# blindopen/TSM-Det-Pointcloud-

Measured on AMD Instinct MI355X. Metric: point-cloud frames/sec (fwd+bwd), higher is better.
Workload: dtype f32; 1 GPU; BASELINE configs[1]: KITTI-shaped synthetic, 20000 pts / 16000 active voxels per frame, full SECOND detector (VoxelBackBone8x) fwd+bwd+AdamW step; batch_per_gpu=4, global_batch=4, parallelism=dp1, voxelize_on_gpu=True

## Files before the change

include/spx.h:

```cpp
#ifndef SPX_H_
#define SPX_H_

#include <stddef.h>
#include <stdint.h>

#ifdef __cplusplus
extern "C" {
#endif

#define SPX_ABI_VERSION 3

#define SPX_OK 0
#define SPX_ERR_INVALID_ARG (-1)
#define SPX_ERR_WORKSPACE (-2)
#define SPX_ERR_UNSUPPORTED (-3)
#define SPX_ERR_LAUNCH (-4)
#define SPX_ERR_TOO_LARGE (-5)
#define SPX_ERR_CAPACITY (-7)
#define SPX_ERR_TABLE_FULL (-6)
#define SPX_ERR_RING_STALL (-8)
#define SPX_ERR_BATCH_STATS (-10)
#define SPX_ERR_OUT_OF_GRID (-9)

#define SPX_WS_PRECLEARED 1
// ... 83 lines not shown
int spx_densify_bwd(const float *ddense, const int32_t *idx, int64_t n, const int64_t *d_n, int c, int batch,
                    const int32_t *shape, int layout, float *dfeat, spx_stream_t stream);

int spx_boxes_iou_bev(const float *boxes_a, int64_t n, const float *boxes_b, int64_t m, int overlap_only, float *out,
                      spx_stream_t stream);
size_t spx_nms_ws_bytes(int64_t n);
int spx_nms_bev(const float *boxes, int64_t n, float thresh, int axis_aligned, int64_t *keep, int64_t *d_num_keep,
                void *ws, size_t ws_bytes, spx_stream_t stream);

size_t spx_assign_targets_ws_bytes(int batch, int n_sets, int max_gt);
int spx_assign_targets(const float *anchors, int n_sets, int64_t anchors_per_set, int per_location,
                       const float *gt_boxes, int batch, int max_gt, const int32_t *d_set_class, int n_classes,
                       const float *d_matched, const float *d_unmatched, int32_t *labels, float *targets,
                       float *weights, void *ws, size_t ws_bytes, spx_stream_t stream);

size_t spx_anchor_loss_ws_bytes(int batch, int64_t n_anchors);
int spx_anchor_loss(const float *cls_preds, const float *box_preds, const float *dir_preds, const int32_t *labels,
                    const float *reg_targets, const float *anchors, int batch, int64_t n_anchors, int num_class,
                    int num_dir_bins, float dir_offset, float cls_weight, float loc_weight, float dir_weight,
                    float beta, float alpha, float *losses, float *dcls, float *dbox, float *ddir, void *ws,
                    size_t ws_bytes, spx_stream_t stream);

size_t spx_bn_relu_ws_bytes(int c);
int spx_bn_relu_fwd(const float *x, int64_t n, const int64_t *d_n, int c, const float *gamma, const float *beta,
                    float *running_mean, float *running_var, float momentum, float eps, int relu, float *y,
                    float *save_mean, float *save_invstd, void *ws, size_t ws_bytes, spx_stream_t stream);
int spx_bn_relu_bwd(const float *x, const float *dy, int64_t n, const int64_t *d_n, int c, const float *gamma, const float *beta,
                    const float *save_mean, const float *save_invstd, int relu, float *dx, float *dgamma, float *dbeta,
                    void *ws, size_t ws_bytes, spx_stream_t stream);

int spx_bn_add_relu_fwd(const float *x, const float *res, int64_t n, const int64_t *d_n, int c, const float *gamma,
                        const float *beta, float *running_mean, float *running_var, int64_t *num_batches_tracked,
                        float momentum, float eps, int relu, float *y, int64_t y_ld, float *save_mean, float *save_invstd,
                        void *ws, size_t ws_bytes, spx_stream_t stream);
int spx_bn_add_relu_bwd(const float *x, const float *res, const float *dy, int64_t dy_ld, int64_t n, const int64_t *d_n,
                        int c, const float *gamma, const float *beta, const float *save_mean, const float *save_invstd, int relu,
                        float *dx, float *dres, float *dgamma, float *dbeta, void *ws, size_t ws_bytes,
                        spx_stream_t stream);

int spx_bn_apply(const float *x, const float *res, int64_t n, const int64_t *d_n, int c, const float *mean,
                 const float *invstd, const float *gamma, const float *beta, int relu, float *y, int64_t y_ld,
                 spx_stream_t stream);

int spx_bn_relu_fwd_from_sums(const float *x, int64_t n, const int64_t *d_n, int c, const float *partial, int64_t nblk,
                              const float *gamma,
                              const float *beta, float *running_mean, float *running_var, int64_t *num_batches_tracked,
                              float momentum, float eps, int relu, float *y, int64_t y_ld, float *save_mean,
                              float *save_invstd, spx_stream_t stream);

int64_t spx_wino_stat_rows(int32_t n, int32_t h, int32_t w);
int64_t spx_wino_weight_floats(int32_t cin, int32_t cout);
int spx_wino_weight(const float *w, int64_t s_o, int64_t s_i, int64_t s_a, int64_t s_b, int32_t cin, int32_t cout, int flip,
                    float *u, spx_stream_t stream);
int spx_conv2d_wino(const float *x, int64_t x_ld, const float *u, int32_t n, int32_t h, int32_t w, int32_t cin, int32_t cout,
                    const float *scale, const float *shift, int relu, float *y, int64_t y_ld, float *stat_partials,
                    spx_stream_t stream);

size_t spx_wino_wgrad_ws_bytes(int32_t cin, int32_t cout);
int spx_conv2d_wino_wgrad(const float *x, int64_t x_ld, const float *dy, int64_t dy_ld, int32_t n, int32_t h, int32_t w,
                          int32_t cin, int32_t cout, float *dw, int64_t s_o, int64_t s_i, int64_t s_a, int64_t s_b, void *ws,
                          size_t ws_bytes, spx_stream_t stream);

int spx_voxel_query(const float *new_xyz, const float *xyz, const int32_t *new_coords, const int32_t *point_indices,
                    int64_t m, int batch, const int32_t *shape3, int nsample, float radius, const int32_t *range3,
                    int32_t *idx, int32_t *cnt_unique, spx_stream_t stream);

int spx_voxel_query_dilated(const float *new_xyz, const float *xyz, const int32_t *new_coords,
                            const int32_t *point_indices, int64_t m, int batch, const int32_t *shape3, int nsample,
                            float former_radius, float radius, const int32_t *range3, const int32_t *stride3,
                            int32_t *idx, int32_t *cnt_unique, int32_t *idx_cnt, spx_stream_t stream);


size_t spx_furthest_point_sample_ws_bytes(int32_t b, int64_t n);
int spx_furthest_point_sample(const float *xyz, const float *weights, int32_t b, int64_t n, int32_t npoint, int32_t *idx,
                              void *ws, size_t ws_bytes, spx_stream_t stream);

size_t spx_furthest_point_sample_matrix_ws_bytes(int32_t b, int64_t n);
int spx_furthest_point_sample_matrix(const float *matrix, const float *weights, int32_t b, int64_t n, int32_t npoint,
                                     int32_t *idx, void *ws, size_t ws_bytes, spx_stream_t stream);

int spx_ball_query(const float *xyz, const float *new_xyz, int32_t b, int64_t n, int64_t m, float r_in, float r_out,
                   int32_t nsample, int32_t *idx_cnt, int32_t *idx, spx_stream_t stream);

int spx_group_points(const float *features, const int32_t *idx, int32_t b, int32_t c, int64_t n, int64_t m,
                     int32_t nsample, float *out, spx_stream_t stream);

size_t spx_group_points_bwd_ws_bytes(int32_t b, int64_t n, int64_t m, int32_t nsample);
int spx_group_points_bwd(const float *grad_out, const int32_t *idx, int32_t b, int32_t c, int64_t n, int64_t m,
                         int32_t nsample, float *grad_features, void *ws, size_t ws_bytes, spx_stream_t stream);

int spx_three_nn(const float *unknown, const float *known, int32_t b, int64_t n, int64_t m, float *dist2, int32_t *idx,
                 spx_stream_t stream);

int spx_three_interpolate(const float *features, const int32_t *idx, const float *weight, int32_t b, int32_t c, int64_t m,
                          int64_t n, float *out, spx_stream_t stream);
size_t spx_three_interpolate_bwd_ws_bytes(int32_t b, int64_t m, int64_t n);
int spx_three_interpolate_bwd(const float *grad_out, const int32_t *idx, const float *weight, int32_t b, int32_t c,
                              int64_t m, int64_t n, float *grad_features, void *ws, size_t ws_bytes, spx_stream_t stream);


int spx_points_in_boxes(const float *pts, const float *boxes, int32_t b, int64_t m, int64_t t, int32_t *box_idx,
                        spx_stream_t stream);

size_t spx_roiaware_pool3d_ws_bytes(int64_t n, int64_t np, int32_t ox, int32_t oy, int32_t oz);
int spx_roiaware_pool3d_fwd(const float *rois, const float *pts, const float *feats, int64_t n, int64_t np, int32_t c,
                            int32_t ox, int32_t oy, int32_t oz, int32_t max_pts, int32_t mode, float *pooled,
// ... 199 lines not shown
```

tsm-det-pointcloud-_amd/csrc/wino_conv2d.hip:

```cpp
#include "spx_common.h"

namespace {

typedef float f32x16 __attribute__((ext_vector_type(16)));
typedef float f32x4 __attribute__((ext_vector_type(4)));
typedef float f32x2 __attribute__((ext_vector_type(2)));
typedef unsigned int u32x4 __attribute__((ext_vector_type(4)));

constexpr int kTiles = 32;
constexpr int kKc = 8;
constexpr int kSc = 16;
constexpr int kCoWg = 128;
constexpr int kThreads = 512;
constexpr int kPosFloats = kCoWg * kKc;
constexpr int kPlane = kTiles * kKc + 8;

struct WinoArgs {
  const float* x;
  const float* u;
  float* y;
  const float* scale;
  const float* shift;
  float* stats;
  int64_t x_ld, y_ld;
  uint32_t x_bytes, u_bytes;
  int32_t n, h, w, cin, cout;
  int32_t tiles_x, tiles_y;
  int64_t n_tiles;
  int32_t relu;
  int32_t n_blocks;
};

constexpr int qp(int a, int b, int c, int d) { return a | (b << 2) | (c << 4) | (d << 6); }

__device__ __forceinline__ float dpp_p(float v) {
  return __builtin_bit_cast(float, __builtin_amdgcn_mov_dpp(__builtin_bit_cast(int, v), qp(0, 1, 2, 1), 0xF, 0xF, true));
}
__device__ __forceinline__ float dpp_q(float v) {
  return __builtin_bit_cast(float, __builtin_amdgcn_mov_dpp(__builtin_bit_cast(int, v), qp(2, 2, 1, 3), 0xF, 0xF, true));
}

__host__ __device__ constexpr int wino_channel(int chunk, int slot) {
  return (chunk >> 1) * kSc + (slot >> 1) * 4 + (chunk & 1) * 2 + (slot & 1);
}

__global__ void k_wino_weight(const float* __restrict__ w, int64_t s_o, int64_t s_i, int64_t s_a, int64_t s_b, int cin,
                              int cout, int flip, float* __restrict__ u) {
  const int64_t idx = (int64_t)blockIdx.x * blockDim.x + threadIdx.x;
  const int64_t total = (int64_t)cin * cout;
  if (idx >= total) return;
  const int nchunk = cin / kKc;
  const int sidx = (int)(idx & 3);
  const int col = (int)((idx >> 2) & 31);
  const int hh = (int)((idx >> 7) & 1);
  const int nb = (int)((idx >> 8) & 3);
  const int chunk = (int)((idx >> 10) % nchunk);
  const int cb = (int)((idx >> 10) / nchunk);
  const int ci = wino_channel(chunk, 4 * hh + sidx), co = cb * kCoWg + nb * 32 + col;
  float g[3][3];
#pragma unroll
  for (int a = 0; a < 3; ++a)
#pragma unroll
    for (int b = 0; b < 3; ++b)
      g[a][b] = flip ? w[(int64_t)ci * s_o + (int64_t)co * s_i + (2 - a) * s_a + (2 - b) * s_b]
                     : w[(int64_t)co * s_o + (int64_t)ci * s_i + a * s_a + b * s_b];
  float t[4][3];
#pragma unroll
  for (int b = 0; b < 3; ++b) {
    t[0][b] = g[0][b];
    t[1][b] = 0.5f * (g[0][b] + g[1][b] + g[2][b]);
    t[2][b] = 0.5f * (g[0][b] - g[1][b] + g[2][b]);
    t[3][b] = g[2][b];
  }
  float* dst = u + ((int64_t)(cb * nchunk + chunk) * 16) * kPosFloats + (idx & 1023);
#pragma unroll
  for (int i = 0; i < 4; ++i) {
    dst[(int64_t)(i * 4 + 0) * kPosFloats] = t[i][0];
    dst[(int64_t)(i * 4 + 1) * kPosFloats] = 0.5f * (t[i][0] + t[i][1] + t[i][2]);
    dst[(int64_t)(i * 4 + 2) * kPosFloats] = 0.5f * (t[i][0] - t[i][1] + t[i][2]);
    dst[(int64_t)(i * 4 + 3) * kPosFloats] = t[i][2];
  }
}

template <int NB>
__global__ void __launch_bounds__(kThreads) __attribute__((amdgpu_waves_per_eu(NB == 1 ? 4 : 2, NB == 1 ? 4 : 2)))
k_wino_conv(WinoArgs a) {
  constexpr int kCoW = 64 * NB;
  constexpr int kSmemFloats = 4 * kTiles * kCoW > 2 * 16 * kPlane ? 4 * kTiles * kCoW : 2 * 16 * kPlane;
  __shared__ __attribute__((aligned(16))) float smem[kSmemFloats];

  const int tid = threadIdx.x;
  const int lane = tid & 63;
  const int wave = tid >> 6;
  const int wrow = wave & 3;
  const int half = wave >> 2;
  const int l31 = lane & 31, lh = lane >> 5;

  const int ncb = a.cout / kCoW;
  const int xcd = blockIdx.x & 7, rest = blockIdx.x >> 3;
  const int per = (a.n_blocks + 7) >> 3;
  const int cbw = rest % ncb;
  const int bid = xcd * per + rest / ncb;
  if (bid >= a.n_blocks) return;
  const int64_t tile0 = (int64_t)bid * kTiles;
  const int nbg = (cbw * 2 + half) * NB;
  const int nchunk = a.cin / kKc;
  const int nsuper = a.cin / kSc;

  const int ld_col = tid & 3;
  const int ld_g = (tid >> 2) & 3;
  const int ld_tile = tid >> 4;
  const __amdgpu_buffer_rsrc_t rs_x =
      __builtin_amdgcn_make_buffer_rsrc(const_cast<float*>(a.x), 0, (int)a.x_bytes, 0x00020000);
  const __amdgpu_buffer_rsrc_t rs_u =
      __builtin_amdgcn_make_buffer_rsrc(const_cast<float*>(a.u), 0, (int)a.u_bytes, 0x00020000);
  uint32_t xoff[4];
  {
    const int64_t t = tile0 + ld_tile;
    const bool tv = t < a.n_tiles;
    const int64_t tt = tv ? t : 0;
    const int tx = (int)(tt % a.tiles_x);
    const int ty = (int)((tt / a.tiles_x) % a.tiles_y);
    const int nn = (int)(tt / ((int64_t)a.tiles_x * a.tiles_y));
    const int px = 2 * tx - 1 + ld_col;
#pragma unroll
    for (int i = 0; i < 4; ++i) {
      const int py = 2 * ty - 1 + i;
      const bool ok = tv && px >= 0 && px < a.w && py >= 0 && py < a.h;
      const int64_t pix = ((int64_t)nn * a.h + py) * a.w + px;
      xoff[i] = ok ? (uint32_t)((pix * a.x_ld + ld_g * 4) * 4) : 0xFFFFFFF0u;
    }
  }
  const float sgn = (ld_col == 1) ? 1.0f : -1.0f;
  float* const vdst = smem + ld_col * kPlane + ld_tile * kKc + ld_g * 2;
// ... 123 lines not shown
        f32x4 y1 = (r1 - r2 - r3) * sc4 + sh4;
        if (a.stats) {
          const float m0 = (px < a.w) ? 1.f : 0.f, m1 = (px < a.w && 2 * ty + 1 < a.h) ? 1.f : 0.f;
          st_s += y0 * m0 + y1 * m1;
          st_q += y0 * y0 * m0 + y1 * y1 * m1;
        }
        if (a.relu) {
#pragma unroll
          for (int e = 0; e < 4; ++e) {
            y0[e] = fmaxf(y0[e], 0.f);
            y1[e] = fmaxf(y1[e], 0.f);
          }
        }
        if (px < a.w) {
          const int py = 2 * ty;
          float* dst = a.y + (((int64_t)nn * a.h + py) * a.w + px) * a.y_ld + co0;
          *reinterpret_cast<f32x4*>(dst) = y0;
          if (py + 1 < a.h) *reinterpret_cast<f32x4*>(dst + (int64_t)a.w * a.y_ld) = y1;
        }
      }
    }
    if (c2 == 0) __syncthreads();
  }
  if (a.stats) {
    __syncthreads();
    float* red = smem;
    *reinterpret_cast<f32x4*>(red + (o_t * kQuads + o_q) * 8) = st_s;
    *reinterpret_cast<f32x4*>(red + (o_t * kQuads + o_q) * 8 + 4) = st_q;
    __syncthreads();
    if (tid < kCoW) {
      const int q = tid >> 2, e = tid & 3;
      float s1 = 0.f, s2 = 0.f;
      for (int t = 0; t < kTilesPass; ++t) {
        s1 += red[(t * kQuads + q) * 8 + e];
        s2 += red[(t * kQuads + q) * 8 + 4 + e];
      }
      float* dst = a.stats + (int64_t)bid * 2 * a.cout + cbw * kCoW + tid;
      dst[0] = s1;
      dst[a.cout] = s2;
    }
  }
}

}

extern "C" int64_t spx_wino_weight_floats(int32_t cin, int32_t cout) { return (int64_t)16 * cin * cout; }

extern "C" int spx_wino_weight(const float* w, int64_t s_o, int64_t s_i, int64_t s_a, int64_t s_b, int32_t cin, int32_t cout,
                               int flip, float* u, spx_stream_t stream) {
  if (cin <= 0 || cout <= 0 || cin % kSc != 0 || cout % kCoWg != 0) return SPX_ERR_INVALID_ARG;
  const int64_t total = (int64_t)cin * cout;
  hipLaunchKernelGGL(k_wino_weight, dim3((unsigned)((total + 255) / 256)), dim3(256), 0, spx_s(stream), w, s_o, s_i, s_a,
                     s_b, cin, cout, flip, u);
  SPX_CHECK_LAUNCH();
  return SPX_OK;
}

extern "C" int64_t spx_wino_stat_rows(int32_t n, int32_t h, int32_t w) {
  const int64_t tiles = (int64_t)n * ((w + 1) / 2) * ((h + 1) / 2);
  return (tiles + kTiles - 1) / kTiles;
}

extern "C" int spx_conv2d_wino(const float* x, int64_t x_ld, const float* u, int32_t n, int32_t h, int32_t w, int32_t cin,
                               int32_t cout, const float* scale, const float* shift, int relu, float* y, int64_t y_ld,
                               float* stat_partials, spx_stream_t stream) {
  if (n <= 0 || h <= 0 || w <= 0) return SPX_OK;
  if (cin % kSc != 0 || cout % kCoWg != 0 || x_ld < cin || y_ld < cout || (x_ld & 3) || (y_ld & 3)) return SPX_ERR_INVALID_ARG;
  const int64_t x_bytes = ((int64_t)n * h * w - 1) * x_ld * 4 + (int64_t)cin * 4, u_bytes = (int64_t)16 * cin * cout * 4;
  if (x_bytes >= 0xFFFFFFF0ll || u_bytes >= 0x7FFFFFFFll) return SPX_ERR_TOO_LARGE;
  WinoArgs a;
  a.x = x; a.u = u; a.y = y; a.scale = scale; a.shift = shift; a.stats = stat_partials;
  a.x_ld = x_ld; a.y_ld = y_ld;
  a.x_bytes = (uint32_t)x_bytes; a.u_bytes = (uint32_t)u_bytes;
  a.n = n; a.h = h; a.w = w; a.cin = cin; a.cout = cout;
  a.tiles_x = (w + 1) / 2; a.tiles_y = (h + 1) / 2;
  a.n_tiles = (int64_t)n * a.tiles_x * a.tiles_y;
  a.relu = relu;
  const int64_t nb = (a.n_tiles + kTiles - 1) / kTiles;
  if (nb > 0x7fffffff) return SPX_ERR_INVALID_ARG;
  a.n_blocks = (int32_t)nb;
#ifdef WINO_FORCE_NB
  const bool narrow = WINO_FORCE_NB == 1;
#else
  const bool narrow = true;
#endif
  const int64_t nb8 = (nb + 7) / 8 * 8;
  if (narrow)
    hipLaunchKernelGGL(k_wino_conv<1>, dim3((unsigned)(nb8 * (cout / 64))), dim3(kThreads), 0, spx_s(stream), a);
  else
    hipLaunchKernelGGL(k_wino_conv<2>, dim3((unsigned)(nb8 * (cout / 128))), dim3(kThreads), 0, spx_s(stream), a);
  SPX_CHECK_LAUNCH();
  return SPX_OK;
}
```

tsm-det-pointcloud-_amd/pcdet_amd/models/backbones_2d/base_bev_backbone.py:

```python
import os

import numpy as np
import torch
import torch.nn as nn
import torch.nn.functional as F

from spx import ops

from ..model_utils import det_wgrad
from spx.functional import (bn_relu_cat_train, bn_relu_train, dense as densify_rows, folded_bn, sparse_conv, wino_conv2d,
                            wino_conv2d_ok, wino_conv_bn_relu_train)

_FUSED_BN_MIN_ELEMS = int(os.environ.get("SPX_BEV_FUSED_BN_MIN", str(8 * 1000 * 1000)))


def _run_block(seq, x, start=0):
    mods = list(seq)
    i = start
    while i < len(mods):
        m = mods[i]
        nxt = mods[i + 1] if i + 1 < len(mods) else None
        if (isinstance(m, nn.ZeroPad2d) and isinstance(nxt, nn.Conv2d) and tuple(nxt.padding) == (0, 0)
                and nxt.padding_mode == 'zeros' and len(set(m.padding)) == 1 and isinstance(nxt.padding, tuple)):
            p = int(m.padding[0])
            if det_wgrad.usable(x, nxt):
                x = det_wgrad.conv2d(x, nxt, p)
            else:
                x = F.conv2d(x, nxt.weight, nxt.bias, nxt.stride, (p, p), nxt.dilation, nxt.groups)
            i += 2
            continue
        if _WINO and isinstance(m, nn.Conv2d) and wino_conv2d_ok(x, m):
            nn2 = mods[i + 2] if i + 2 < len(mods) else None
            if (_CONV_BN_NODE and isinstance(nxt, nn.BatchNorm2d) and isinstance(nn2, nn.ReLU) and _train_bn_ok(nxt)
                    and torch.is_grad_enabled()
                    and x.shape[0] * x.shape[2] * x.shape[3] * m.out_channels >= _FUSED_BN_MIN_ELEMS
                    and 1024 % m.out_channels == 0):
                x = wino_conv_bn_relu_train(x, m, nxt)
                i += 3
            elif nxt is not None and isinstance(nn2, nn.ReLU) and _eval_bn_ok(nxt, x, check_layout=False):
                scale, shift, _ = folded_bn(nxt)
                x = wino_conv2d(x, m.weight, scale=scale, shift=shift, relu=True)
                i += 3
            else:
                x = wino_conv2d(x, m.weight)
                i += 1
            continue
        if (isinstance(m, nn.BatchNorm2d) and isinstance(nxt, nn.ReLU) and m.training and m.affine
                and m.track_running_stats and m.momentum is not None and x.is_cuda and x.dtype == torch.float32
                and x.numel() >= _FUSED_BN_MIN_ELEMS and 1024 % x.shape[1] == 0 and x.shape[1] % 4 == 0
                and x.is_contiguous(memory_format=torch.channels_last)):
            b, c, h, w = x.shape
            y = bn_relu_train(x.permute(0, 2, 3, 1).reshape(b * h * w, c), m, True)
            x = y.view(b, h, w, c).permute(0, 3, 1, 2)
            i += 2
            continue
        if _eval_bn_ok(m, x) and isinstance(nxt, nn.ReLU):
            b, c, h, w = x.shape
            y = _bn_eval_rows(x.permute(0, 2, 3, 1).reshape(b * h * w, c), m, True)
            x = y.view(b, h, w, c).permute(0, 3, 1, 2)
            i += 2
            continue
        x = _up(m, x) if isinstance(m, nn.ConvTranspose2d) else m(x)
        i += 1
    return x


def _up(m, x):
    return det_wgrad.conv_transpose2d(x, m) if det_wgrad.usable(x, m) else m(x)


_FUSED_EVAL_BN = os.environ.get("SPX_BEV_FUSED_EVAL_BN", "1") != "0"


_WINO = os.environ.get("SPX_BEV_WINOGRAD", "1") != "0"
_CONV_BN_NODE = os.environ.get("SPX_BEV_CONV_BN_NODE", "1") != "0"


def _train_bn_ok(m):
    return m.training and m.affine and m.track_running_stats and m.momentum is not None and m.weight.dtype == torch.float32


def _eval_bn_ok(m, x, check_layout=True):
    return (_FUSED_EVAL_BN and isinstance(m, nn.BatchNorm2d) and not m.training and m.affine and m.running_mean is not None
            and not torch.is_grad_enabled() and x.is_cuda and x.dtype == torch.float32 and x.dim() == 4
            and not torch.is_autocast_enabled()
            and (not check_layout or (1024 % x.shape[1] == 0 and x.shape[1] % 4 == 0
                                      and x.is_contiguous(memory_format=torch.channels_last))))


def _bn_eval_rows(rows, bn, relu, out=None):
    _scale, _shift, invstd = folded_bn(bn)
    return ops.bn_apply(rows, bn.running_mean, invstd, bn.weight, bn.bias, relu, out=out)


_SPARSE_ENTRY = os.environ.get("SPX_BEV_SPARSE_ENTRY", "1") != "0"
_FUSED_CAT = os.environ.get("SPX_BEV_FUSED_CAT", "1") != "0"
_WIDE_BALANCED = os.environ.get("SPX_BEV_WIDE_BALANCED", "1") != "0"
_SPARSE_ENTRY_CHANNELS = (16, 32, 64, 128)


def _sparse_entry(seq, bev):
    tag = getattr(bev, '_spx_source', None)
    mods = list(seq)
    if not _SPARSE_ENTRY or tag is None or tag[1] != bev._version or len(mods) < 2:
        return None
    src = tag[0]
    pad, conv = mods[0], mods[1]
    if not (isinstance(pad, nn.ZeroPad2d) and isinstance(conv, nn.Conv2d) and len(set(pad.padding)) == 1
            and tuple(conv.padding) == (0, 0) and conv.padding_mode == 'zeros' and conv.bias is None and conv.groups == 1
            and tuple(conv.dilation) == (1, 1) and conv.stride[0] == conv.stride[1]):
        return None
    feats = src.features
    c, d = feats.shape[1], int(src.spatial_shape[0])
    kh, kw = conv.kernel_size
    if not (feats.is_cuda and feats.dtype == torch.float32 and bev.dtype == torch.float32
            and not torch.is_autocast_enabled() and conv.in_channels == c * d and d * kh * kw <= 30
            and c in _SPARSE_ENTRY_CHANNELS and conv.out_channels in _SPARSE_ENTRY_CHANNELS and feats.shape[0] > 0):
# ... 36 lines not shown
        self.blocks = nn.ModuleList()
        self.deblocks = nn.ModuleList()
        for idx in range(num_levels):
            c_out = num_filters[idx]
            layers = [nn.ZeroPad2d(1),
                      nn.Conv2d(c_in_list[idx], c_out, kernel_size=3, stride=layer_strides[idx], padding=0, bias=False),
                      bn(c_out), nn.ReLU()]
            for _ in range(layer_nums[idx]):
                layers += [nn.Conv2d(c_out, c_out, kernel_size=3, padding=1, bias=False), bn(c_out), nn.ReLU()]
            self.blocks.append(nn.Sequential(*layers))
            if len(upsample_strides) > 0:
                stride = upsample_strides[idx]
                if stride >= 1:
                    up = nn.ConvTranspose2d(c_out, num_upsample_filters[idx], stride, stride=stride, bias=False)
                else:
                    s = int(np.round(1 / stride))
                    up = nn.Conv2d(c_out, num_upsample_filters[idx], s, stride=s, bias=False)
                self.deblocks.append(nn.Sequential(up, bn(num_upsample_filters[idx]), nn.ReLU()))

        c_in = sum(num_upsample_filters)
        if len(upsample_strides) > num_levels:
            self.deblocks.append(nn.Sequential(
                nn.ConvTranspose2d(c_in, c_in, upsample_strides[-1], stride=upsample_strides[-1], bias=False),
                bn(c_in), nn.ReLU()))
        self.num_bev_features = c_in
        self.num_voxel_neck_features = c_in
        self.num_point_features = kwargs.get('num_point_features', None)

    def _cat_fusable(self):
        if not _FUSED_CAT or len(self.deblocks) != len(self.blocks) or len(self.deblocks) < 2:
            return False
        for d in self.deblocks:
            mods = list(d)
            if not (len(mods) == 3 and isinstance(mods[1], nn.BatchNorm2d) and isinstance(mods[2], nn.ReLU)
                    and mods[1].training and mods[1].affine and mods[1].track_running_stats and mods[1].momentum is not None
                    and 1024 % mods[1].num_features == 0 and mods[1].num_features % 4 == 0):
                return False
        return True

    def _cat_eval_fusable(self, x):
        if not _FUSED_EVAL_BN or len(self.deblocks) != len(self.blocks) or len(self.deblocks) < 2 or torch.is_grad_enabled():
            return False
        return all(len(d) == 3 and isinstance(d[1], nn.BatchNorm2d) and isinstance(d[2], nn.ReLU) and not d[1].training
                   and d[1].affine and d[1].running_mean is not None and 1024 % d[1].num_features == 0
                   and d[1].num_features % 4 == 0 for d in self.deblocks)

    def forward(self, data_dict):
        spatial_features = data_dict['spatial_features']
        ups, pre = [], []
        x = spatial_features
        plain = x.is_cuda and x.dtype == torch.float32 and not torch.is_autocast_enabled()
        fuse_cat = self._cat_fusable() and plain
        fuse_cat_eval = (not fuse_cat) and plain and self._cat_eval_fusable(x)
        for i in range(len(self.blocks)):
            y = _sparse_entry(self.blocks[i], x) if i == 0 else None
            x = _run_block(self.blocks[i], x) if y is None else _run_block(self.blocks[i], y, start=2)
            stride = int(spatial_features.shape[2] / x.shape[2])
            data_dict['spatial_features_%dx' % stride] = x
            if fuse_cat or fuse_cat_eval:
                pre.append(_up(self.deblocks[i][0], x))
            else:
                ups.append(_run_block(self.deblocks[i], x) if len(self.deblocks) > 0 else x)
        if fuse_cat or fuse_cat_eval:
            b, _c, h, w = pre[0].shape
            same = all(t.shape[0] == b and t.shape[2:] == pre[0].shape[2:]
                       and t.is_contiguous(memory_format=torch.channels_last) for t in pre)
            if same and fuse_cat and all(t.numel() >= _FUSED_BN_MIN_ELEMS for t in pre):
                rows = [t.permute(0, 2, 3, 1).reshape(b * h * w, t.shape[1]) for t in pre]
                y = bn_relu_cat_train(rows, [d[1] for d in self.deblocks])
                ups = [y.view(b, h, w, y.shape[1]).permute(0, 3, 1, 2)]
            elif same and fuse_cat_eval:
                widths = [t.shape[1] for t in pre]
                y = torch.empty((b * h * w, sum(widths)), dtype=torch.float32, device=x.device)
                off = 0
                for t, d, wd in zip(pre, self.deblocks, widths):
                    _bn_eval_rows(t.permute(0, 2, 3, 1).reshape(b * h * w, wd), d[1], True, out=y[:, off:off + wd])
                    off += wd
                ups = [y.view(b, h, w, y.shape[1]).permute(0, 3, 1, 2)]
            else:
                ups = [_run_block(d, t, start=1) for d, t in zip(self.deblocks, pre)]
        if len(ups) > 1:
            x = torch.cat(ups, dim=1)
        elif len(ups) == 1:
            x = ups[0]
        if len(self.deblocks) > len(self.blocks):
            x = _run_block(self.deblocks[-1], x)
        data_dict['spatial_features_2d'] = x
        data_dict['encoded_bev_features'] = [x]
        return data_dict
```

tsm-det-pointcloud-_amd/spx/_lib.py:

```python
import ctypes
import os

import torch

_HERE = os.path.dirname(os.path.abspath(__file__))
LIB_PATH = os.environ.get("SPX_LIB_PATH") or os.path.join(os.path.dirname(_HERE), "csrc", "libspx.so")

SPX_ABI_VERSION = 3
SPX_MAX_KVOL = 32

_vp = ctypes.c_void_p
_i64 = ctypes.c_int64
_int = ctypes.c_int
_sz = ctypes.c_size_t
_i32p = ctypes.POINTER(ctypes.c_int32)
_f32p = ctypes.POINTER(ctypes.c_float)
_vpp = ctypes.POINTER(ctypes.c_void_p)

class PointMlp(ctypes.Structure):
    _fields_ = [("w1", _vp), ("bn_mean", _vp), ("bn_var", _vp), ("bn_weight", _vp), ("bn_bias", _vp),
                ("bn_eps", ctypes.c_float), ("w2", _vp), ("b2", _vp)]


_mlpp = ctypes.POINTER(PointMlp)
# ... 5 lines not shown
    "spx_read_status": (_int, [_vp, _vp]),
    "spx_voxelize": (_int, [_vp, _i64, _int, _int, _int, _int, _int, _int, _f32p, _f32p, _i32p, _int, _int, _vp, _vp,
                            _vp, _vp, _vp, _i64, _int, _vp, _vp, _sz, _vp]),
    "spx_dynamic_voxelize_ws_bytes": (_sz, [_i64, _int, _i32p, _i64]),
    "spx_dynamic_voxelize": (_int, [_vp, _i64, _int, _int, _int, _int, _f32p, _f32p, _i32p, _int, _vp, _vp, _vp, _vp, _i64,
                                    _vp, _sz, _vp]),
    "spx_voxel_query": (_int, [_vp, _vp, _vp, _vp, _i64, _int, _i32p, _int, ctypes.c_float, _i32p, _vp, _vp, _vp]),
    "spx_voxel_query_dilated": (_int, [_vp, _vp, _vp, _vp, _i64, _int, _i32p, _int, ctypes.c_float, ctypes.c_float, _i32p,
                                       _i32p, _vp, _vp, _vp, _vp]),
    "spx_mean_vfe": (_int, [_vp, _vp, _i64, _vp, _int, _int, _vp, _vp]),
    "spx_subm_rulebook_ws_bytes": (_sz, [_i64]),
    "spx_subm_rulebook": (_int, [_vp, _i64, _vp, _int, _i32p, _i32p, _i32p, _vp, _i64, _vp, _int, _vp, _vp, _sz, _vp]),
    "spx_conv_out_cap": (_i64, [_i64, _int, _i32p, _i32p, _i32p]),
    "spx_conv_rulebook_ws_bytes": (_sz, [_i64, _int, _i32p]),
    "spx_conv_rulebook": (_int, [_vp, _i64, _vp, _int, _i32p, _i32p, _i32p, _i32p, _i32p, _i32p, _vp, _vp, _vp, _vp,
                                 _vp, _i64, _i32p, _i32p, _vp, _vp, _vp, _vp, _sz, _vp]),
    "spx_pack_weight": (_int, [_vp, _int, _int, _int, _int, _vp, _vp]),
    "spx_pack_weight_batched": (_int, [_vp, _int, _i64, _vp]),
    "spx_conv_gemm": (_int, [_vp, _int, _vp, _int, _int, _int, _vp, _i64, _i64, _vp, _vp, _vp, _int, _vp, _vp]),
    "spx_conv_plan_bytes": (_sz, [_i64]),
    "spx_conv_plan": (_int, [_vp, _i64, _int, _i64, _vp, _vp, _vp]),
    "spx_conv_gemm_balanced_ws_bytes": (_sz, [_int, _i64]),
    "spx_conv_group_ws_bytes": (_sz, [_i64]),
    "spx_conv_group": (_int, [_vp, _i64, _int, _i64, _vp, _vp, _vp, _vp, _sz, _vp]),
    "spx_conv_gemm_balanced": (_int, [_vp, _int, _vp, _int, _int, _int, _vp, _i64, _i64, _vp, _vp, _vp, _int, _vp, _vp, _vp,
                                      _vp, _sz, _vp]),
    "spx_conv_ring_plan_bytes": (_sz, [_i64]),
    "spx_conv_ring_stat_rows": (_int, []),
    "spx_conv_ring_tiles_per_wave": (_int, [_int]),
    "spx_conv_ring_plan": (_int, [_vp, _i64, _int, _i64, _vp, _vp, _vp]),
    "spx_conv_gemm_ring": (_int, [_vp, _i64, _int, _vp, _int, _int, _int, _vp, _i64, _i64, _vp, _vp, _vp, _int, _vp, _vp, _vp,
                                  _vp, _vp, _vp]),
    "spx_conv_wgrad_ws_bytes": (_sz, [_int, _int, _int, _i64]),
    "spx_conv_wgrad_counts_bytes": (_sz, [_int, _i64]),
    "spx_conv_wgrad_counts": (_int, [_vp, _i64, _int, _i64, _vp, _vp, _vp]),
    "spx_conv_wgrad": (_int, [_vp, _int, _vp, _int, _int, _vp, _i64, _i64, _vp, _vp, _vp, _vp, _sz, _vp]),
    "spx_densify": (_int, [_vp, _vp, _i64, _vp, _int, _int, _i32p, _int, _vp, _vp]),
    "spx_densify_bwd": (_int, [_vp, _vp, _i64, _vp, _int, _int, _i32p, _int, _vp, _vp]),
    "spx_boxes_iou_bev": (_int, [_vp, _i64, _vp, _i64, _int, _vp, _vp]),
    "spx_nms_ws_bytes": (_sz, [_i64]),
    "spx_nms_bev": (_int, [_vp, _i64, ctypes.c_float, _int, _vp, _vp, _vp, _sz, _vp]),
    "spx_assign_targets_ws_bytes": (_sz, [_int, _int, _int]),
    "spx_bn_relu_ws_bytes": (_sz, [_int]),
    "spx_bn_relu_fwd": (_int, [_vp, _i64, _vp, _int, _vp, _vp, _vp, _vp, ctypes.c_float, ctypes.c_float, _int, _vp, _vp,
                               _vp, _vp, _sz, _vp]),
    "spx_bn_relu_bwd": (_int, [_vp, _vp, _i64, _vp, _int, _vp, _vp, _vp, _vp, _int, _vp, _vp, _vp, _vp, _sz, _vp]),
    "spx_bn_add_relu_fwd": (_int, [_vp, _vp, _i64, _vp, _int, _vp, _vp, _vp, _vp, _vp, ctypes.c_float, ctypes.c_float, _int,
                                   _vp, _i64, _vp, _vp, _vp, _sz, _vp]),
    "spx_bn_add_relu_bwd": (_int, [_vp, _vp, _vp, _i64, _i64, _vp, _int, _vp, _vp, _vp, _vp, _int, _vp, _vp, _vp, _vp, _vp, _sz,
                                   _vp]),
    "spx_bn_apply": (_int, [_vp, _vp, _i64, _vp, _int, _vp, _vp, _vp, _vp, _int, _vp, _i64, _vp]),
    "spx_wino_weight_floats": (_i64, [_int, _int]),
    "spx_wino_weight": (_int, [_vp, _i64, _i64, _i64, _i64, _int, _int, _int, _vp, _vp]),
    "spx_conv2d_wino": (_int, [_vp, _i64, _vp, _int, _int, _int, _int, _int, _vp, _vp, _int, _vp, _i64, _vp, _vp]),
    "spx_wino_stat_rows": (_i64, [_int, _int, _int]),
    "spx_bn_relu_fwd_from_sums": (_int, [_vp, _i64, _vp, _int, _vp, _i64, _vp, _vp, _vp, _vp, _vp, ctypes.c_float, ctypes.c_float,
                                         _int, _vp, _i64, _vp, _vp, _vp]),
    "spx_wino_wgrad_ws_bytes": (_sz, [_int, _int]),
    "spx_conv2d_wino_wgrad": (_int, [_vp, _i64, _vp, _i64, _int, _int, _int, _int, _int, _vp, _i64, _i64, _i64, _i64, _vp, _sz,
                                     _vp]),
    "spx_anchor_loss_ws_bytes": (_sz, [_int, _i64]),
    "spx_anchor_loss": (_int, [_vp, _vp, _vp, _vp, _vp, _vp, _int, _i64, _int, _int, ctypes.c_float, ctypes.c_float,
                               ctypes.c_float, ctypes.c_float, ctypes.c_float, ctypes.c_float, _vp, _vp, _vp, _vp, _vp, _sz,
                               _vp]),
    "spx_assign_targets": (_int, [_vp, _int, _i64, _int, _vp, _int, _int, _vp, _int, _vp, _vp, _vp, _vp, _vp, _vp, _sz,
                                  _vp]),
    "spx_furthest_point_sample_ws_bytes": (_sz, [ctypes.c_int32, _i64]),
    "spx_furthest_point_sample": (_int, [_vp, _vp, ctypes.c_int32, _i64, ctypes.c_int32, _vp, _vp, _sz, _vp]),
    "spx_furthest_point_sample_matrix_ws_bytes": (_sz, [ctypes.c_int32, _i64]),
    "spx_furthest_point_sample_matrix": (_int, [_vp, _vp, ctypes.c_int32, _i64, ctypes.c_int32, _vp, _vp, _sz, _vp]),
    "spx_ball_query": (_int, [_vp, _vp, ctypes.c_int32, _i64, _i64, ctypes.c_float, ctypes.c_float, ctypes.c_int32, _vp,
                              _vp, _vp]),
    "spx_group_points": (_int, [_vp, _vp, ctypes.c_int32, ctypes.c_int32, _i64, _i64, ctypes.c_int32, _vp, _vp]),
    "spx_group_points_bwd_ws_bytes": (_sz, [ctypes.c_int32, _i64, _i64, ctypes.c_int32]),
    "spx_group_points_bwd": (_int, [_vp, _vp, ctypes.c_int32, ctypes.c_int32, _i64, _i64, ctypes.c_int32, _vp, _vp, _sz,
                                    _vp]),
    "spx_three_nn": (_int, [_vp, _vp, ctypes.c_int32, _i64, _i64, _vp, _vp, _vp]),
    "spx_three_interpolate": (_int, [_vp, _vp, _vp, ctypes.c_int32, ctypes.c_int32, _i64, _i64, _vp, _vp]),
    "spx_three_interpolate_bwd_ws_bytes": (_sz, [ctypes.c_int32, _i64, _i64]),
    "spx_three_interpolate_bwd": (_int, [_vp, _vp, _vp, ctypes.c_int32, ctypes.c_int32, _i64, _i64, _vp, _vp, _sz, _vp]),
    "spx_points_in_boxes": (_int, [_vp, _vp, ctypes.c_int32, _i64, _i64, _vp, _vp]),
    "spx_roiaware_pool3d_ws_bytes": (_sz, [_i64, _i64, ctypes.c_int32, ctypes.c_int32, ctypes.c_int32]),
    "spx_roiaware_pool3d_fwd": (_int, [_vp, _vp, _vp, _i64, _i64, ctypes.c_int32, ctypes.c_int32, ctypes.c_int32,
                                       ctypes.c_int32, ctypes.c_int32, ctypes.c_int32, _vp, _vp, _vp, _vp, _vp, _sz, _vp]),
    "spx_roiaware_pool3d_bwd": (_int, [_vp, _vp, _vp, _vp, _i64, _i64, ctypes.c_int32, ctypes.c_int32, ctypes.c_int32,
                                       ctypes.c_int32, ctypes.c_int32, _vp, _vp]),
    "spx_group_project": (_int, [_vp, _vp, _vp, _vp, _vp, _vp, ctypes.c_int32, _i64, ctypes.c_int32, _i64, ctypes.c_int32,
                                 _vp, _vp]),
    "spx_group_project_bwd_ws_bytes": (_sz, [ctypes.c_int32, _i64, ctypes.c_int32, _i64, ctypes.c_int32]),
    "spx_group_project_bwd": (_int, [_vp, _vp, _vp, _vp, _vp, ctypes.c_int32, _i64, ctypes.c_int32, _i64, ctypes.c_int32,
                                     _vp, _vp, _vp, _sz, _vp]),
    "spx_point_vote": (_int, [_vp, _vp, ctypes.c_int32, ctypes.c_int32, _i64, _i64, _i64, _mlpp, ctypes.c_int32, _f32p,
                              _vp, _vp]),
    "spx_point_head_predict": (_int, [_vp, _vp, _vp, ctypes.c_int32, ctypes.c_int32, _i64, ctypes.c_int32, _mlpp,
                                      ctypes.c_int32, _mlpp, ctypes.c_int32, ctypes.c_int32, _vp, _vp, _vp, _vp]),
    "spx_point_post_process_capacity": (_i64, [_i64, ctypes.c_int32, _i64, _int]),
    "spx_point_post_process_ws_bytes": (_sz, [ctypes.c_int32, _i64, ctypes.c_int32, _i64]),
    "spx_point_post_process": (_int, [_vp, _vp, _vp, ctypes.c_int32, _i64, _f32p, ctypes.c_int32, ctypes.c_float, _i64,
                                      _i64, _int, _int, _vp, _vp, _vp, _vp, _vp, _vp, _sz, _vp]),
    "spx_recall_count": (_int, [_vp, _vp, ctypes.c_int32, _i64, _vp, _i64, ctypes.c_int32, _f32p, ctypes.c_int32, _vp,
                                _vp, _vp]),
    "spx_point_assign_targets": (_int, [_vp, _vp, ctypes.c_int32, _i64, _i64, ctypes.c_int32, _f32p, ctypes.c_int32,
                                        ctypes.c_float, ctypes.c_int32, ctypes.c_int32, _vp, _vp, _vp, _vp, _vp, _vp,
                                        _vp]),
    "spx_point_head_loss_ws_bytes": (_sz, [_i64]),
    "spx_point_head_loss": (_int, [_vp] * 12 + [_i64, ctypes.c_int32, ctypes.c_int32, _f32p, _int, _int, _int, _vp, _vp,
# ... 101 lines not shown
```

tsm-det-pointcloud-_amd/spx/functional.py:

```python
import os
import weakref

import torch

from . import ops


def _packed(weight, mode):
    if weight.is_cuda and torch.cuda.is_current_stream_capturing():
        if not torch.is_grad_enabled():
            holder = weight._base if weight._base is not None else weight
            hit = (getattr(holder, "_spx_packed", None) or {}).get(
                (mode, weight.data_ptr(), tuple(weight.shape), tuple(weight.stride())))
            if hit is not None and hit[0] == weight._version:
                return _graph_constant(weight, hit[1], lambda w, out, mode=mode: ops.pack_weight(w, mode, out=out))
        return ops.pack_weight(weight, mode)
    holder = weight._base if weight._base is not None else weight
    cache = getattr(holder, "_spx_packed", None)
    if cache is None:
        cache = {}
        try:
            holder._spx_packed = cache
        except AttributeError:
            return ops.pack_weight(weight, mode)
# ... 369 lines not shown
def bn_relu_cat_train(xs, bns):
    moms = tuple(bn.momentum for bn in bns)
    epss = tuple(bn.eps for bn in bns)
    args = (tuple(xs) + tuple(bn.weight for bn in bns) + tuple(bn.bias for bn in bns) + tuple(bn.running_mean for bn in bns)
            + tuple(bn.running_var for bn in bns) + tuple(bn.num_batches_tracked for bn in bns))
    return _BNReLUCatFn.apply(moms, epss, *args)


def bn_momentum_ok(bn):
    return bn.momentum is not None


def bn_train_fusable(bn, f):
    return (isinstance(bn, torch.nn.BatchNorm1d) and bn.training and bn.affine and bn.track_running_stats
            and bn_momentum_ok(bn) and f.is_cuda
            and f.dtype == torch.float32 and f.dim() == 2 and f.shape[0] > 1 and ops.bn_relu_supported(f.shape[1]))


def bn_relu_train(x, bn, relu, residual=None, d_n=None):
    return _BNReLUFn.apply(x, bn.weight, bn.bias, bn.running_mean, bn.running_var, bn.momentum, bn.eps, relu, residual,
                           bn.num_batches_tracked, d_n)


def bn_act(x, bn, relu, residual=None, d_n=None):
    if bn_train_fusable(bn, x):
        return bn_relu_train(x, bn, relu, residual, d_n)
    if d_n is not None:
        if bn.training or bn.running_mean is None:
            raise RuntimeError("static-capacity rows need the fused BatchNorm kernels (training mode on the GPU, fp32) or a "
                               "BatchNorm on its running statistics")
        live = (torch.arange(x.shape[0], device=x.device) < d_n).unsqueeze(1)
        zero = torch.zeros((), dtype=x.dtype, device=x.device)
        y = bn(torch.where(live, x, zero))
        if residual is not None:
            y = y + torch.where(live, residual, zero)
        y = torch.relu(y) if relu else y
        return torch.where(live, y, zero)
    y = bn(x)
    if residual is not None:
        y = y + residual
    return torch.relu(y) if relu else y


def _wino_image(weight, flip):
    if weight.is_cuda and torch.cuda.is_current_stream_capturing():
        hit = getattr(weight, '_spx_wino_flip' if flip else '_spx_wino', None)
        if (not torch.is_grad_enabled() and hit is not None and hit[0] == weight._version and hit[1] == weight.data_ptr()
                and hit[2].device == weight.device):
            return _graph_constant(weight, hit[2], lambda w, out, flip=flip: ops.wino_weight(w, flip, out=out))
        return ops.wino_weight(weight, flip)
    attr = '_spx_wino_flip' if flip else '_spx_wino'
    hit = getattr(weight, attr, None)
    fresh = hit is not None and hit[1] == weight.data_ptr() and hit[2].device == weight.device
    if fresh and hit[0] == weight._version and not (torch.is_grad_enabled() and weight.requires_grad):
        return hit[2]
    u = ops.wino_weight(weight, flip, out=hit[2] if fresh else None)
    setattr(weight, attr, (weight._version, weight.data_ptr(), u))
    return u


def _wino_image_always(weight, flip):
    with torch.enable_grad():
        return _wino_image(weight, flip)


def wino_conv2d_ok(x, conv):
    return (x.is_cuda and x.dtype == torch.float32 and x.dim() == 4 and not torch.is_autocast_enabled()
            and tuple(conv.kernel_size) == (3, 3) and tuple(conv.stride) == (1, 1) and conv.padding == (1, 1)
            and tuple(conv.dilation) == (1, 1) and conv.groups == 1 and conv.bias is None and conv.padding_mode == 'zeros'
            and conv.weight.dtype == torch.float32 and ops.wino_ok(conv.in_channels, conv.out_channels)
            and x.shape[1] == conv.in_channels and ops._cl_ld(x) is not None)


_WINO_WGRAD = os.environ.get("SPX_BEV_WINOGRAD_WGRAD", "1") != "0"
class _WinoConv2dFn(torch.autograd.Function):

    @staticmethod
    def forward(ctx, x, weight):
        ctx.save_for_backward(x, weight)
        return ops.conv2d_wino(x, _wino_image(weight, False), weight.shape[0])

    @staticmethod
    def backward(ctx, dy):
        x, weight = ctx.saved_tensors
        return _wino_backward(x, weight, dy, ctx.needs_input_grad[0], ctx.needs_input_grad[1])


def _wino_backward(x, weight, dy, needs_x, needs_w):
    dx = dw = None
    if ops._cl_ld(dy) is None:
        dy = dy.contiguous(memory_format=torch.channels_last)
    if needs_x:
        if ops.wino_ok(weight.shape[0], weight.shape[1]):
            dx = ops.conv2d_wino(dy, _wino_image_always(weight, True), weight.shape[1])
        else:
            dx = torch.ops.aten.convolution_backward(dy, x, weight, None, (1, 1), (1, 1), (1, 1), False, (0, 0), 1,
                                                     (True, False, False))[0]
    if needs_w:
        if _WINO_WGRAD and ops.wino_wgrad_ok(weight.shape[1], weight.shape[0], x.shape[3]):
            if _ASYNC_WGRAD:
                dw = _off_critical_path(lambda: ops.conv2d_wino_wgrad(x, dy, weight), [x, dy], weight)
            else:
                dw = ops.conv2d_wino_wgrad(x, dy, weight)
        else:
            dw = torch.ops.aten.convolution_backward(dy, x, weight, None, (1, 1), (1, 1), (1, 1), False, (0, 0), 1,
                                                     (False, True, False))[1]
    return dx, dw


class _WinoConvBNReLUFn(torch.autograd.Function):

# ... 34 lines not shown
```

tsm-det-pointcloud-_amd/spx/ops.py:

```python
import ctypes
import os

import torch

from . import _lib
from ._lib import check, f_arr, i3

_WS = {}


_raw_stream = getattr(torch._C, "_cuda_getCurrentRawStream", None)


def _stream_handle(device):
    if _raw_stream is not None:
        idx = device.index
        return _raw_stream(torch.cuda.current_device() if idx is None else idx)
    return torch.cuda.current_stream(device).cuda_stream


def _stream(t):
    return ctypes.c_void_p(_stream_handle(t.device))


# ... 616 lines not shown
    _need_gpu(x, partial, gamma, beta)
    lib = _lib.load()
    x = x.contiguous()
    n, c = x.shape
    assert partial.dim() == 3 and partial.shape[1] == 2 and partial.shape[2] == c and partial.is_contiguous()
    y = torch.empty_like(x)
    mean = torch.empty((c,), dtype=torch.float32, device=x.device)
    invstd = torch.empty((c,), dtype=torch.float32, device=x.device)
    check(lib.spx_bn_relu_fwd_from_sums(_ptr(x), n, _ptr(d_n), c, _ptr(partial), int(partial.shape[0]), _ptr(gamma), _ptr(beta),
                                        _ptr(running_mean), _ptr(running_var), _ptr(num_batches_tracked), float(momentum),
                                        float(eps), int(bool(relu)), _ptr(y), c, _ptr(mean), _ptr(invstd), _stream(x)),
          "spx_bn_relu_fwd_from_sums")
    return y, mean, invstd


def bn_apply(x, mean, invstd, gamma, beta, relu, residual=None, out=None, d_n=None):
    _need_gpu(x, mean, invstd, gamma, beta)
    lib = _lib.load()
    x = x.contiguous()
    n, c = x.shape
    if out is None:
        y = torch.empty_like(x)
    else:
        if not (_row_view_ok(out, n, c) and out.device == x.device):
            raise ValueError("out must be a float32 [N, C] row view (row stride a multiple of 4, 16-byte aligned)")
        y = out
    y_ld = y.stride(0) if n > 1 else c
    if residual is not None:
        residual = residual.contiguous()
    check(lib.spx_bn_apply(_ptr(x), _ptr(residual), n, _ptr(d_n), c, _ptr(mean), _ptr(invstd), _ptr(gamma), _ptr(beta),
                           int(bool(relu)), _ptr(y), y_ld, _stream(x)), "spx_bn_apply")
    return y


def wino_ok(cin, cout):
    return cin % 32 == 0 and cout % 128 == 0


def wino_weight(weight, flip=False, out=None):
    _need_gpu(weight)
    assert weight.dim() == 4 and weight.shape[2] == 3 and weight.shape[3] == 3 and weight.dtype == torch.float32
    lib = _lib.load()
    cout, cin = int(weight.shape[0]), int(weight.shape[1])
    k_in, k_out = (cout, cin) if flip else (cin, cout)
    nfl = lib.spx_wino_weight_floats(k_in, k_out)
    if out is not None and out.numel() == nfl and out.device == weight.device and out.dtype == torch.float32:
        u = out
    else:
        u = torch.empty((nfl,), dtype=torch.float32, device=weight.device)
    so, si, sa, sb = weight.stride()
    check(lib.spx_wino_weight(_ptr(weight), so, si, sa, sb, k_in, k_out, int(bool(flip)), _ptr(u), _stream(weight)),
          "spx_wino_weight")
    return u


def conv2d_wino(x, u, cout, scale=None, shift=None, relu=False, out=None, stats=False):
    _need_gpu(x, u)
    lib = _lib.load()
    n, cin, h, w = (int(v) for v in x.shape)
    x_ld = _cl_ld(x)
    if x_ld is None:
        x = x.contiguous(memory_format=torch.channels_last)
        x_ld = _cl_ld(x)
    if out is None:
        out = torch.empty((n, cout, h, w), dtype=torch.float32, device=x.device, memory_format=torch.channels_last)
    y_ld = _cl_ld(out)
    if y_ld is None or tuple(out.shape) != (n, cout, h, w):
        raise ValueError("out must be a float32 [N, Cout, H, W] channels-last map")
    if u.numel() != lib.spx_wino_weight_floats(cin, cout):
        raise ValueError("weight image does not match Cin=%d, Cout=%d" % (cin, cout))
    part = None
    if stats:
        part = torch.empty((lib.spx_wino_stat_rows(n, h, w), 2, cout), dtype=torch.float32, device=x.device)
    check(lib.spx_conv2d_wino(_ptr(x), x_ld, _ptr(u), n, h, w, cin, cout, _ptr(scale), _ptr(shift), int(bool(relu)),
                              _ptr(out), y_ld, _ptr(part), _stream(x)), "spx_conv2d_wino")
    return (out, part) if stats else out


def wino_wgrad_ok(cin, cout, w):
    return cin % 128 == 0 and cout % 128 == 0 and (w + 1) // 2 >= 8


def conv2d_wino_wgrad(x, dy, like):
    _need_gpu(x, dy)
    lib = _lib.load()
    n, cin, h, w = (int(v) for v in x.shape)
    cout = int(dy.shape[1])
    x_ld, dy_ld = _cl_ld(x), _cl_ld(dy)
    if x_ld is None:
        x = x.contiguous(memory_format=torch.channels_last)
        x_ld = _cl_ld(x)
    if dy_ld is None:
        dy = dy.contiguous(memory_format=torch.channels_last)
        dy_ld = _cl_ld(dy)
    assert tuple(like.shape) == (cout, cin, 3, 3) and tuple(dy.shape) == (n, cout, h, w)
    dw = torch.empty_like(like)
    so, si, sa, sb = dw.stride()
    wsb = lib.spx_wino_wgrad_ws_bytes(cin, cout)
    ws = workspace(x.device, wsb)
    check(lib.spx_conv2d_wino_wgrad(_ptr(x), x_ld, _ptr(dy), dy_ld, n, h, w, cin, cout, _ptr(dw), so, si, sa, sb, _ptr(ws), wsb,
                                    _stream(x)), "spx_conv2d_wino_wgrad")
    return dw


def _cl_ld(t):
    if t.dtype != torch.float32 or t.dim() != 4:
# ... 1261 lines not shown
```

Before: 294.3 frames/s.

## Batch Winograd weight transforms into one launch on a side stream

Adds a batched weight-transform kernel that uses a device-side job descriptor table and a binary search over block offsets. It builds the forward and flipped Winograd weight images for every eligible conv in a BEV block in a single launch. The launch runs on a side stream at block entry, and the main stream waits on an event before the images are used. This replaces many small per-conv transform launches and overlaps them with other work, at the cost of cache bookkeeping, a persistent bank buffer and cross-stream synchronisation.

Result: no change. 294.6 frames/s (median of 6 runs) (+0.1%).

```diff
diff --git a/include/spx.h b/include/spx.h
--- a/include/spx.h
+++ b/include/spx.h
@@ -159,6 +159,7 @@
 int64_t spx_wino_weight_floats(int32_t cin, int32_t cout);
 int spx_wino_weight(const float *w, int64_t s_o, int64_t s_i, int64_t s_a, int64_t s_b, int32_t cin, int32_t cout, int flip,
                     float *u, spx_stream_t stream);
+int spx_wino_weight_batched(const int64_t *d_desc, int32_t n_jobs, int64_t total_blocks, spx_stream_t stream);
 int spx_conv2d_wino(const float *x, int64_t x_ld, const float *u, int32_t n, int32_t h, int32_t w, int32_t cin, int32_t cout,
                     const float *scale, const float *shift, int relu, float *y, int64_t y_ld, float *stat_partials,
                     spx_stream_t stream);
diff --git a/tsm-det-pointcloud-_amd/csrc/wino_conv2d.hip b/tsm-det-pointcloud-_amd/csrc/wino_conv2d.hip
--- a/tsm-det-pointcloud-_amd/csrc/wino_conv2d.hip
+++ b/tsm-det-pointcloud-_amd/csrc/wino_conv2d.hip
@@ -44,11 +44,8 @@
   return (chunk >> 1) * kSc + (slot >> 1) * 4 + (chunk & 1) * 2 + (slot & 1);
 }
 
-__global__ void k_wino_weight(const float* __restrict__ w, int64_t s_o, int64_t s_i, int64_t s_a, int64_t s_b, int cin,
-                              int cout, int flip, float* __restrict__ u) {
-  const int64_t idx = (int64_t)blockIdx.x * blockDim.x + threadIdx.x;
-  const int64_t total = (int64_t)cin * cout;
-  if (idx >= total) return;
+__device__ __forceinline__ void wino_weight_pair(const float* __restrict__ w, int64_t s_o, int64_t s_i, int64_t s_a,
+                                                 int64_t s_b, int cin, int flip, float* __restrict__ u, int64_t idx) {
   const int nchunk = cin / kKc;
   const int sidx = (int)(idx & 3);
   const int col = (int)((idx >> 2) & 31);
@@ -80,6 +77,28 @@
     dst[(int64_t)(i * 4 + 2) * kPosFloats] = 0.5f * (t[i][0] - t[i][1] + t[i][2]);
     dst[(int64_t)(i * 4 + 3) * kPosFloats] = t[i][2];
   }
+}
+
+__global__ void k_wino_weight(const float* __restrict__ w, int64_t s_o, int64_t s_i, int64_t s_a, int64_t s_b, int cin,
+                              int cout, int flip, float* __restrict__ u) {
+  const int64_t idx = (int64_t)blockIdx.x * blockDim.x + threadIdx.x;
+  if (idx >= (int64_t)cin * cout) return;
+  wino_weight_pair(w, s_o, s_i, s_a, s_b, cin, flip, u, idx);
+}
+
+constexpr int kWinoDescWords = 10;
+__global__ __launch_bounds__(256) void k_wino_weight_batched(const int64_t* __restrict__ desc, int n_jobs) {
+  int lo = 0, hi = n_jobs - 1;
+  while (lo < hi) {
+    const int mid = (lo + hi + 1) >> 1;
+    if (desc[kWinoDescWords * mid + 9] <= (int64_t)blockIdx.x) lo = mid; else hi = mid - 1;
+  }
+  const int64_t* d = desc + kWinoDescWords * lo;
+  const int cin = (int)d[5], cout = (int)d[6];
+  const int64_t idx = ((int64_t)blockIdx.x - d[9]) * 256 + threadIdx.x;
+  if (idx < 0 || idx >= (int64_t)cin * cout) return;
+  wino_weight_pair(reinterpret_cast<const float*>(d[0]), d[1], d[2], d[3], d[4], cin, (int)d[7],
+                   reinterpret_cast<float*>(d[8]), idx);
 }
 
 template <int NB>
@@ -309,6 +328,14 @@
   const int64_t total = (int64_t)cin * cout;
   hipLaunchKernelGGL(k_wino_weight, dim3((unsigned)((total + 255) / 256)), dim3(256), 0, spx_s(stream), w, s_o, s_i, s_a,
                      s_b, cin, cout, flip, u);
+  SPX_CHECK_LAUNCH();
+  return SPX_OK;
+}
+
+extern "C" int spx_wino_weight_batched(const int64_t* d_desc, int32_t n_jobs, int64_t total_blocks, spx_stream_t stream) {
+  if (!d_desc || n_jobs <= 0 || total_blocks <= 0) return SPX_ERR_INVALID_ARG;
+  if (total_blocks >= (int64_t(1) << 31)) return SPX_ERR_TOO_LARGE;
+  hipLaunchKernelGGL(k_wino_weight_batched, dim3((unsigned)total_blocks), dim3(256), 0, spx_s(stream), d_desc, n_jobs);
   SPX_CHECK_LAUNCH();
   return SPX_OK;
 }
diff --git a/tsm-det-pointcloud-_amd/pcdet_amd/models/backbones_2d/base_bev_backbone.py b/tsm-det-pointcloud-_amd/pcdet_amd/models/backbones_2d/base_bev_backbone.py
--- a/tsm-det-pointcloud-_amd/pcdet_amd/models/backbones_2d/base_bev_backbone.py
+++ b/tsm-det-pointcloud-_amd/pcdet_amd/models/backbones_2d/base_bev_backbone.py
@@ -9,7 +9,7 @@
 
 from ..model_utils import det_wgrad
 from spx.functional import (bn_relu_cat_train, bn_relu_train, dense as densify_rows, folded_bn, sparse_conv, wino_conv2d,
-                            wino_conv2d_ok, wino_conv_bn_relu_train)
+                            wino_conv2d_ok, wino_conv_bn_relu_train, wino_conv_module_ok, wino_images_all)
 
 _FUSED_BN_MIN_ELEMS = int(os.environ.get("SPX_BEV_FUSED_BN_MIN", str(8 * 1000 * 1000)))
 
@@ -17,6 +17,7 @@
 def _run_block(seq, x, start=0):
     mods = list(seq)
     i = start
+    _queue_wino_images(seq, x)
     while i < len(mods):
         m = mods[i]
         nxt = mods[i + 1] if i + 1 < len(mods) else None
@@ -63,6 +64,16 @@
         x = _up(m, x) if isinstance(m, nn.ConvTranspose2d) else m(x)
         i += 1
     return x
+
+
+def _queue_wino_images(module, x):
+    if not (_WINO and x.is_cuda and x.dtype == torch.float32 and torch.is_grad_enabled()
+            and not torch.is_autocast_enabled()):
+        return
+    convs = getattr(module, '_spx_wino_convs', None)
+    if convs is None:
+        convs = module._spx_wino_convs = [m for m in module.modules() if wino_conv_module_ok(m)]
+    wino_images_all(convs)
 
 
 def _up(m, x):
@@ -205,6 +216,7 @@
         plain = x.is_cuda and x.dtype == torch.float32 and not torch.is_autocast_enabled()
         fuse_cat = self._cat_fusable() and plain
         fuse_cat_eval = (not fuse_cat) and plain and self._cat_eval_fusable(x)
+        _queue_wino_images(self, x)
         for i in range(len(self.blocks)):
             y = _sparse_entry(self.blocks[i], x) if i == 0 else None
             x = _run_block(self.blocks[i], x) if y is None else _run_block(self.blocks[i], y, start=2)
diff --git a/tsm-det-pointcloud-_amd/spx/_lib.py b/tsm-det-pointcloud-_amd/spx/_lib.py
--- a/tsm-det-pointcloud-_amd/spx/_lib.py
+++ b/tsm-det-pointcloud-_amd/spx/_lib.py
@@ -81,6 +81,7 @@
     "spx_bn_apply": (_int, [_vp, _vp, _i64, _vp, _int, _vp, _vp, _vp, _vp, _int, _vp, _i64, _vp]),
     "spx_wino_weight_floats": (_i64, [_int, _int]),
     "spx_wino_weight": (_int, [_vp, _i64, _i64, _i64, _i64, _int, _int, _int, _vp, _vp]),
+    "spx_wino_weight_batched": (_int, [_vp, _int, _i64, _vp]),
     "spx_conv2d_wino": (_int, [_vp, _i64, _vp, _int, _int, _int, _int, _int, _vp, _vp, _int, _vp, _i64, _vp, _vp]),
     "spx_wino_stat_rows": (_i64, [_int, _int, _int]),
     "spx_bn_relu_fwd_from_sums": (_int, [_vp, _i64, _vp, _int, _vp, _i64, _vp, _vp, _vp, _vp, _vp, ctypes.c_float, ctypes.c_float,
diff --git a/tsm-det-pointcloud-_amd/spx/functional.py b/tsm-det-pointcloud-_amd/spx/functional.py
--- a/tsm-det-pointcloud-_amd/spx/functional.py
+++ b/tsm-det-pointcloud-_amd/spx/functional.py
@@ -445,11 +445,85 @@
     attr = '_spx_wino_flip' if flip else '_spx_wino'
     hit = getattr(weight, attr, None)
     fresh = hit is not None and hit[1] == weight.data_ptr() and hit[2].device == weight.device
-    if fresh and hit[0] == weight._version and not (torch.is_grad_enabled() and weight.requires_grad):
-        return hit[2]
+    if weight.is_cuda:
+        _wino_bank_wait(weight.device)
+    if fresh and hit[0] == weight._version:
+        if not (torch.is_grad_enabled() and weight.requires_grad):
+            return hit[2]
+        if _WINO_BANK and len(hit) > 3 and hit[3]:
+            setattr(weight, attr, hit[:3] + (False,))
+            return hit[2]
     u = ops.wino_weight(weight, flip, out=hit[2] if fresh else None)
-    setattr(weight, attr, (weight._version, weight.data_ptr(), u))
+    setattr(weight, attr, (weight._version, weight.data_ptr(), u, False))
     return u
+
+
+_WINO_BANK = os.environ.get("SPX_WINO_BANK", "1") != "0"
+_WINO_BANKS = weakref.WeakKeyDictionary()
+_WINO_READY = {}
+
+
+def _wino_bank_wait(device):
+    ev = _WINO_READY.pop(device.index, None) if _WINO_READY else None
+    if ev is not None:
+        torch.cuda.current_stream(device).wait_event(ev)
+
+
+def _wino_stale(weight, flip):
+    hit = getattr(weight, '_spx_wino_flip' if flip else '_spx_wino', None)
+    if hit is None or hit[0] != weight._version or hit[1] != weight.data_ptr() or hit[2].device != weight.device:
+        return True
+    return flip and weight.requires_grad and not (len(hit) > 3 and hit[3])
+
+
+def wino_conv_module_ok(conv):
+    return (isinstance(conv, torch.nn.Conv2d) and tuple(conv.kernel_size) == (3, 3) and tuple(conv.stride) == (1, 1)
+            and conv.padding == (1, 1) and tuple(conv.dilation) == (1, 1) and conv.groups == 1 and conv.bias is None
+            and conv.padding_mode == 'zeros' and ops.wino_ok(conv.in_channels, conv.out_channels))
+
+
+def wino_images_all(convs):
+    if not _WINO_BANK or not convs:
+        return 0
+    ws, seen = [], set()
+    for m in convs:
+        w = m.weight
+        if w.is_cuda and w.dtype == torch.float32 and id(w) not in seen:
+            seen.add(id(w))
+            ws.append(w)
+    if not ws or torch.cuda.is_current_stream_capturing():
+        return 0
+    fwd_stale = any(_wino_stale(w, False) for w in ws if ops.wino_ok(w.shape[1], w.shape[0]))
+    if not fwd_stale and not any(_wino_stale(w, True) for w in ws if ops.wino_ok(w.shape[0], w.shape[1])):
+        return 0
+    from .prebuild import side_stream
+    banks = _WINO_BANKS.get(convs[0])
+    if banks is None:
+        banks = _WINO_BANKS[convs[0]] = {}
+    key = ops.WinoBank.geometry(ws)
+    bank = banks.get(key)
+    if bank is None:
+        if len(banks) >= 4:
+            banks.clear()
+        bank = banks[key] = ops.WinoBank(ws)
+        bank.flat.record_stream(side_stream(ws[0].device))
+    dev = ws[0].device
+    main, side = torch.cuda.current_stream(dev), side_stream(dev)
+    side.wait_stream(main)
+    with torch.cuda.stream(side):
+        n = bank.fill(flipped_only=not fwd_stale)
+        ready = torch.cuda.Event()
+        ready.record(side)
+    _WINO_READY[dev.index] = ready
+    for w, (u_fwd, u_flip) in zip(ws, bank.images):
+        try:
+            if u_fwd is not None and fwd_stale:
+                w._spx_wino = (w._version, w.data_ptr(), u_fwd, True)
+            if u_flip is not None:
+                w._spx_wino_flip = (w._version, w.data_ptr(), u_flip, True)
+        except AttributeError:
+            pass
+    return n
 
 
 def _wino_image_always(weight, flip):
diff --git a/tsm-det-pointcloud-_amd/spx/ops.py b/tsm-det-pointcloud-_amd/spx/ops.py
--- a/tsm-det-pointcloud-_amd/spx/ops.py
+++ b/tsm-det-pointcloud-_amd/spx/ops.py
@@ -692,6 +692,69 @@
     check(lib.spx_wino_weight(_ptr(weight), so, si, sa, sb, k_in, k_out, int(bool(flip)), _ptr(u), _stream(weight)),
           "spx_wino_weight")
     return u
+
+
+def wino_weight_batched(desc, n_jobs, total_blocks):
+    _need_gpu(desc)
+    assert desc.dtype == torch.int64 and desc.is_contiguous() and 0 < n_jobs <= desc.shape[0]
+    check(_lib.load().spx_wino_weight_batched(_ptr(desc), int(n_jobs), int(total_blocks), _stream(desc)),
+          "spx_wino_weight_batched")
+
+
+def wino_bank_jobs(weights):
+    jobs, off, blk = [], 0, 0
+    n_flip = flip_blocks = 0
+    for flip in (True, False):
+        for i, w in enumerate(weights):
+            assert w.dim() == 4 and w.shape[2] == 3 and w.shape[3] == 3
+            cout, cin = int(w.shape[0]), int(w.shape[1])
+            k_in, k_out = (cout, cin) if flip else (cin, cout)
+            if not wino_ok(k_in, k_out):
+                continue
+            jobs.append(dict(weight=i, flip=flip, cin=k_in, cout=k_out, strides=tuple(int(s) for s in w.stride()),
+                             offset=off, first_block=blk))
+            off += 16 * k_in * k_out
+            blk += k_in * k_out // 256
+        if flip:
+            n_flip, flip_blocks = len(jobs), blk
+    return jobs, n_flip, flip_blocks, blk, off
+
+
+class WinoBank(object):
+
+    def __init__(self, weights, flat=None):
+        self.weights = list(weights)
+        dev = self.weights[0].device
+        _need_gpu(*self.weights)
+        assert all(w.dtype == torch.float32 and w.device == dev for w in self.weights)
+        self.jobs, self.n_flip, self.flip_blocks, self.blocks, floats = wino_bank_jobs(self.weights)
+        if flat is None:
+            flat = torch.empty((floats,), dtype=torch.float32, device=dev)
+        assert flat.dtype == torch.float32 and flat.is_contiguous() and flat.device == dev and flat.numel() >= floats
+        self.flat = flat
+        self.images = [[None, None] for _ in self.weights]
+        rows = []
+        for j in self.jobs:
+            w = self.weights[j["weight"]]
+            n = 16 * j["cin"] * j["cout"]
+            u = flat[j["offset"]:j["offset"] + n]
+            self.images[j["weight"]][1 if j["flip"] else 0] = u
+            rows.append([w.data_ptr(), *j["strides"], j["cin"], j["cout"], int(j["flip"]), u.data_ptr(), j["first_block"]])
+        self.desc = torch.tensor(rows, dtype=torch.int64).reshape(len(rows), 10).to(dev)
+        self.key = self.geometry(self.weights)
+
+    @staticmethod
+    def geometry(weights):
+        return tuple((w.data_ptr(), tuple(w.shape), tuple(w.stride())) for w in weights)
+
+    def valid_for(self, weights):
+        return self.geometry(weights) == self.key
+
+    def fill(self, flipped_only=False):
+        n, blocks = (self.n_flip, self.flip_blocks) if flipped_only else (len(self.jobs), self.blocks)
+        if n > 0:
+            wino_weight_batched(self.desc, n, blocks)
+        return n
 
 
 def conv2d_wino(x, u, cout, scale=None, shift=None, relu=False, out=None, stats=False):
```
